# sunshinnnn/DSMnet

Measured on AMD Instinct MI355X. Metric: stereo pairs/sec forward, PSMNet D=192 384×1280, at 1/2/4/8 MI355X, higher is better.
Workload: dtype f32

## Files before the change

### dsmnet_amd/_lib.py

```python
import ctypes
import os

_HERE = os.path.dirname(os.path.abspath(__file__))
LIB_PATH = os.environ.get("DSM_LIB_PATH") or os.path.join(_HERE, "csrc", "libdsmnet_hip.so")

c_int, c_void_p, c_size_t = ctypes.c_int, ctypes.c_void_p, ctypes.c_size_t

DSM_OK = 0
DSM_F32 = 0
DSM_NCDHW, DSM_NDHWC = 0, 1
DSM_CONV_FP32_MFMA, DSM_CONV_COUT1_CHUNKED, DSM_CONV_TM_SHIFT, DSM_CONV_BLOCKS_SHIFT = 1, 2, 4, 16
DSM_CONV_NO_NSPLIT = 4
DSM_CONV_NO_ONCE = 8
DSM_PREC_F32, DSM_PREC_F16, DSM_PREC_F16X2 = 0, 1, 2


class Bn3dArgs(ctypes.Structure):
    _fields_ = [("y", c_void_p), ("residual", c_void_p), ("out", c_void_p), ("gamma", c_void_p),
                ("beta", c_void_p), ("running_mean", c_void_p), ("running_var", c_void_p),
                ("affine", c_void_p), ("workspace", c_void_p), ("gout", c_void_p), ("dy", c_void_p),
                ("dresidual", c_void_p), ("B", c_int), ("C", c_int),
                ("Dy", c_int), ("Hy", c_int), ("Wy", c_int), ("Dr", c_int), ("Hr", c_int), ("Wr", c_int),
                ("relu", c_int), ("momentum", ctypes.c_float), ("eps", ctypes.c_float),
                ("out_amax", c_void_p), ("dy_amax", c_void_p), ("dres_amax", c_void_p)]


class Conv3dArgs(ctypes.Structure):
    _fields_ = [("x", c_void_p), ("w_packed", c_void_p), ("scale", c_void_p),
                ("shift", c_void_p), ("residual", c_void_p), ("y", c_void_p),
                ("B", c_int), ("Cin", c_int), ("Cout", c_int),
                ("Di", c_int), ("Hi", c_int), ("Wi", c_int),
                ("Do", c_int), ("Ho", c_int), ("Wo", c_int),
                ("Dr", c_int), ("Hr", c_int), ("Wr", c_int),
                ("stride", c_int), ("transposed", c_int), ("relu", c_int),
                ("kd", c_int), ("k", c_int), ("dil", c_int),
                ("flags", c_int), ("precision", c_int), ("x_amax", c_void_p), ("y_amax", c_void_p),
                ("vol_virtual", c_int), ("vol_mask_left", c_int)]


class BasicBlock2dArgs(ctypes.Structure):
    _fields_ = [("x", c_void_p), ("y", c_void_p), ("w1_packed", c_void_p), ("w2_packed", c_void_p),
                ("scale1", c_void_p), ("shift1", c_void_p), ("scale2", c_void_p), ("shift2", c_void_p),
                ("x_amax", c_void_p), ("y_amax", c_void_p),
                ("B", c_int), ("H", c_int), ("W", c_int), ("C", c_int), ("precision", c_int), ("relu", c_int), ("no_skip", c_int)]


# ... 72 lines not shown
```

### dsmnet_amd/csrc/build.py

```python
import os
import subprocess
import sys
from concurrent.futures import ThreadPoolExecutor

HERE = os.path.dirname(os.path.abspath(__file__))
SOURCES = ["abi.hip", "corr1d.hip", "cost_volume.hip", "soft_argmin.hip", "conv3d.hip", "conv_f16.hip",
           "conv3d_bwd.hip", "bn3d.hip", "decoder.hip", "spp.hip", "warp.hip"]
LIB = os.path.join(HERE, "libdsmnet_hip.so")
HIPCC = os.environ.get("HIPCC", "/opt/rocm/bin/hipcc")
FLAGS = ["--offload-arch=gfx950", "-O3", "-std=c++17", "-fPIC",
         "-Wall", "-Wno-unused-function"] + os.environ.get("HIPCC_EXTRA", "").split()


def _stale(out, deps):
    if not os.path.exists(out):
        return True
    t = os.path.getmtime(out)
    return any(os.path.getmtime(d) > t for d in deps)


def build(force=False, verbose=True, stamps=False):
    if stamps:
        lib = os.path.join(HERE, "libdsmnet_hip_stamps.so")
        srcs = [os.path.join(HERE, s) for s in SOURCES]
        extra = ["-DDSM_ABLATE=%s" % os.environ["DSM_ABLATE"]] if os.environ.get("DSM_ABLATE") else []
        cmd = [HIPCC] + FLAGS + ["-DDSM_STAMPS"] + extra + ["-shared", "-o", lib] + srcs
        print(" ".join(cmd), flush=True)
        subprocess.run(cmd, check=True)
        return lib
    hdrs = [os.path.join(HERE, "common.hpp"), os.path.join(HERE, "conv_split.hpp"), os.path.join(HERE, "conv_zs.hpp"), os.path.join(HERE, "conv_common.hpp"),
            os.path.join(HERE, "..", "..", "include", "dsmnet_hip.h")]
    srcs = [os.path.join(HERE, s) for s in SOURCES if os.path.exists(os.path.join(HERE, s))]
    objs = []
    jobs = []
    for s in srcs:
        o = s[:-4] + ".o"
        objs.append(o)
        if force or _stale(o, [s] + hdrs):
            jobs.append([HIPCC] + FLAGS + ["-c", s, "-o", o])

    def run(cmd):
        if verbose:
            print(" ".join(cmd), flush=True)
        r = subprocess.run(cmd, capture_output=True, text=True)
        if r.returncode != 0:
            raise RuntimeError("hipcc failed:\n%s\n%s" % (r.stdout, r.stderr))
        if verbose and r.stderr.strip():
            print(r.stderr)

    with ThreadPoolExecutor(max_workers=min(4, max(1, len(jobs)))) as ex:
        list(ex.map(run, jobs))
    if jobs or force or _stale(LIB, objs):
        run([HIPCC, "--offload-arch=gfx950", "-shared", "-fPIC", "-o", LIB] + objs)
    return LIB


if __name__ == "__main__":
    print(build(force="--force" in sys.argv, stamps="--stamps" in sys.argv))
```

### dsmnet_amd/csrc/conv3d.hip

```cpp
#include "conv_common.hpp"

#ifdef DSM_STAMPS
__device__ unsigned long long dsm_stamp_buf[8 * 1024];
#define DSM_STAMP(slot)                                                                  \
  do {                                                                                   \
    __builtin_amdgcn_sched_barrier(0);                                                   \
    unsigned long long _t;                                                               \
    asm volatile("s_memtime %0\n\ts_waitcnt lgkmcnt(0)" : "=s"(_t)::"memory");           \
    __builtin_amdgcn_sched_barrier(0);                                                   \
    if (threadIdx.x == 0 && blockIdx.x < 1024) dsm_stamp_buf[blockIdx.x * 8 + (slot)] += _t - _tprev; \
    _tprev = _t;                                                                         \
  } while (0)
#define DSM_STAMP_INIT()                                                                 \
  unsigned long long _tprev;                                                             \
  asm volatile("s_memtime %0\n\ts_waitcnt lgkmcnt(0)" : "=s"(_tprev)::"memory")
extern "C" int dsm_debug_read_stamps(unsigned long long* host, int zero) {
  if (hipMemcpyFromSymbol(host, HIP_SYMBOL(dsm_stamp_buf), sizeof(unsigned long long) * 8 * 1024) != hipSuccess) return -3;
  if (zero) {
    static unsigned long long z[8 * 1024];
    if (hipMemcpyToSymbol(HIP_SYMBOL(dsm_stamp_buf), z, sizeof(z)) != hipSuccess) return -3;
  }
  return 0;
}
#else
// ... 895 lines not shown
    return DSM_OK;
  }
  if (a->stride == 2 && kd == 3 && NT == 2 && bf16x3_enabled(a) &&
      4l * a->B * a->Di * a->Hi * a->Wi * a->Cin < 0x80000000l) {
    *pl = Plan{5, 2, 2, 1, 16, 3, 3, 1};
    return DSM_OK;
  }
fp32_kernels:
  if (kd == 1) {
    const int TM = (big && NT == 1 && a->stride == 1 && k == 3 && dil == 1) ? 2 : 1;
    *pl = Plan{0, a->stride, NT, TM, 16, 1, k, dil};
    return DSM_OK;
  }
  if (a->stride == 1) {
    const int force_tm = forced_tm(a) <= 2 ? forced_tm(a) : 0;
    const int TM = force_tm ? force_tm : ((big && NT <= 2) ? 2 : 1);
    *pl = Plan{0, 1, NT, TM, (NT == 2 && TM == 2) ? 8 : 16, 3, 3, 1};
  } else {
    *pl = Plan{0, 2, NT, 1, 8, 3, 3, 1};
  }
  const long tiles4 = (long)a->B * a->Do * dsm_cdiv(a->Ho, 4) * dsm_cdiv(a->Wo, 32);
  if (NT >= 2 && tiles4 <= 64 && pl->TM == 1) { pl->nsplit = NT; pl->NT = 1; }
  return DSM_OK;
}
int make_plan(const dsm_conv3d_args* a, Plan* pl) {
  const int rc = make_plan_f32(a, pl);
  if (rc != DSM_OK) return rc;
  pl->pm = 3;
  if ((pl->kind == 5 || pl->kind == 6 || pl->kind == 7) && a->precision != DSM_PREC_F32) {
    DSM_REQUIRE(a->x_amax != nullptr, DSM_ERR_ARG);
    pl->pm = a->precision == DSM_PREC_F16X2 ? 2 : 1;
  }
  if (pl->pm == 3) pl->once = 0;
  return DSM_OK;
}
}

extern "C" int dsm_conv3d_plan(const dsm_conv3d_args* a, char* buf, int len) {
  DSM_REQUIRE(buf && len > 0, DSM_ERR_ARG);
  Plan pl;
  int rc = make_plan(a, &pl);
  if (rc != DSM_OK) { buf[0] = 0; return rc; }
  switch (pl.kind) {
    case 0:
      if (pl.KZ == 3 && pl.nsplit > 1) snprintf(buf, len, "conv3d_mfma_kernel<S=%d,NT=%d,TM=%d,CK=%d>x%d", pl.S, pl.NT, pl.TM, pl.CK, pl.nsplit);
      else if (pl.KZ == 3) snprintf(buf, len, "conv3d_mfma_kernel<S=%d,NT=%d,TM=%d,CK=%d>", pl.S, pl.NT, pl.TM, pl.CK);
      else snprintf(buf, len, "conv2d_mfma_kernel<S=%d,NT=%d,TM=%d,K=%d,DIL=%d>", pl.S, pl.NT, pl.TM, pl.K, pl.DIL);
      break;
    case 1: snprintf(buf, len, "deconv3d_mfma_kernel<NT=%d,CK=%d>", pl.NT, pl.CK); break;
    case 2: snprintf(buf, len, "conv3d_cout1_kernel<CK=%d>", pl.CK); break;
    case 4: snprintf(buf, len, "conv3d_cout1_zslide_kernel"); break;
    case 5: {
      const char* pr = pl.pm == 3 ? "bf16x3" : (pl.pm == 2 ? "f16x2" : "f16");
      if (pl.KZ == 3 && pl.S == 2) snprintf(buf, len, "conv3d_%s_mfma_kernel<S=2,NT=%d,TM=%d>", pr, pl.NT, pl.TM);
      else if (pl.KZ == 3 && pl.nsplit > 1) snprintf(buf, len, "conv3d_%s_mfma_kernel<NT=%d,TM=%d>x%d", pr, pl.NT, pl.TM, pl.nsplit);
      else if (pl.KZ == 3) snprintf(buf, len, "conv3d_%s_mfma_kernel<NT=%d,TM=%d>", pr, pl.NT, pl.TM);
      else if (pl.once) snprintf(buf, len, "conv2d_%s_mfma_kernel<NT=%d,TM=%d,DIL=%d>x%d,once", pr, pl.NT, pl.TM, pl.DIL, pl.nsplit);
      else if (pl.nsplit > 1) snprintf(buf, len, "conv2d_%s_mfma_kernel<NT=%d,TM=%d,DIL=%d>x%d", pr, pl.NT, pl.TM, pl.DIL, pl.nsplit);
      else snprintf(buf, len, "conv2d_%s_mfma_kernel<NT=%d,TM=%d,DIL=%d>", pr, pl.NT, pl.TM, pl.DIL);
      break;
    }
    case 7: snprintf(buf, len, "conv3d_zs_%s_mfma_kernel%s", pl.pm == 3 ? "bf16x3" : (pl.pm == 2 ? "f16x2" : "f16"), a->vol_virtual ? "<vol>" : ""); break;
    case 6: snprintf(buf, len, "deconv3d_%s_mfma_kernel<NT=%d>", pl.pm == 3 ? "bf16x3" : (pl.pm == 2 ? "f16x2" : "f16"), pl.NT); break;
    default: snprintf(buf, len, "deconv3d_cout1_kernel"); break;
  }
  return DSM_OK;
}

extern "C" int dsm_basicblock2d_fwd(const dsm_basicblock2d_args* a, dsm_stream_t stream) {
  DSM_REQUIRE(a && a->x && a->y && a->w1_packed && a->w2_packed && a->x_amax, DSM_ERR_ARG);
  DSM_REQUIRE((a->C == 64 || a->C == 32) && a->B > 0 && a->H > 0 && a->W > 0, DSM_ERR_UNSUPPORTED);
  DSM_REQUIRE(a->precision == DSM_PREC_F16X2 || a->precision == DSM_PREC_F16, DSM_ERR_UNSUPPORTED);
  DSM_REQUIRE(a->relu == 0 || a->relu == 1, DSM_ERR_ARG);
  const int C = a->C;
  const unsigned long xb = 4ul * a->B * a->H * a->W * C;
  DSM_REQUIRE(xb < 0x80000000ul, DSM_ERR_UNSUPPORTED);
  const size_t sec3 = (size_t)C * C * 9 * 4 + bf16x3_section_bytes(C, C, 1, 3);
  BbParams p;
  p.x = (const float*)a->x; p.y = (float*)a->y;
  p.w1_amax = (const float*)((const char*)a->w1_packed + sec3);
  p.w2_amax = (const float*)((const char*)a->w2_packed + sec3);
  p.w1 = (const unsigned char*)a->w1_packed + sec3 + 16;
  p.w2 = (const unsigned char*)a->w2_packed + sec3 + 16;
  p.scale1 = a->scale1; p.shift1 = a->shift1; p.scale2 = a->scale2; p.shift2 = a->shift2;
  p.x_amax = a->x_amax; p.y_amax = a->y_amax;
  p.B = a->B; p.H = a->H; p.W = a->W; p.C = C; p.relu = a->relu; p.skip = a->no_skip ? 0 : 1; p.ntx = p.nty = p.ntiles = 0;
  p.xbytes = (unsigned)xb;
  p.wbytes = (unsigned)(f16_section_bytes(C, C, 1, 3) - 16);
  dsm_clear_stale_error();
  return dsmk::run_basicblock_f16(a->precision == DSM_PREC_F16X2 ? 2 : 1, p, (hipStream_t)stream);
}

extern "C" int dsm_conv3d_fwd(const dsm_conv3d_args* a, dsm_stream_t stream) {
  Plan pl;
  int rc = make_plan(a, &pl);
  if (rc != DSM_OK) return rc;
// ... 12 lines not shown
    const size_t n = (size_t)a->Cin * 32 * 27;
    const char* sec2 = (const char*)a->w_packed + n * 4;
    const char* sec3 = sec2 + n * 6;
    z.x = (const float*)a->x; z.scale = a->scale; z.shift = a->shift; z.res = (const float*)a->residual;
    z.y = (float*)a->y; z.x_amax = a->x_amax; z.y_amax = a->y_amax;
    z.w_amax = pl.pm == 3 ? nullptr : (const float*)sec3;
    z.w = (const unsigned char*)(pl.pm == 3 ? sec2 : sec3 + 16);
    z.wbytes = (unsigned)(pl.pm == 3 ? n * 6 : n * 4);
    z.B = a->B; z.Cin = a->Cin;
    z.Di = a->Di; z.Hi = a->Hi; z.Wi = a->Wi; z.Do = a->Do; z.Ho = a->Ho; z.Wo = a->Wo;
    z.Dr = a->Dr; z.Hr = a->Hr; z.Wr = a->Wr; z.relu = a->relu;
    z.vol = a->vol_virtual ? 1 : 0; z.vol_mask_left = a->vol_mask_left ? 1 : 0;
    dsm_clear_stale_error();
    if (pl.pm == 3) return launch_conv_zs<3>(z, p.force_blocks, (hipStream_t)stream);
    return dsmk::run_zs_f16(pl.pm, z, p.force_blocks, (hipStream_t)stream);
  }
  {
    const unsigned long xb = 4ul * a->B * a->Di * a->Hi * a->Wi * a->Cin;
    const int kd_ = a->kd ? a->kd : 3, k_ = a->k ? a->k : 3;
    const unsigned long wb = 4ul * a->Cin * a->Cout * kd_ * k_ * k_;
    DSM_REQUIRE(xb < (1ul << 32) && wb < (1ul << 32), DSM_ERR_UNSUPPORTED);
    p.xbytes = (unsigned)xb; p.wbytes = (unsigned)wb;
  }
  hipStream_t s = (hipStream_t)stream;
  dsm_clear_stale_error();
  if (pl.kind == 3) {
    p.ntx = dsm_cdiv(p.Wi, 32); p.nty = dsm_cdiv(p.Hi, 4);
    const long nt = (long)p.B * p.Di * p.nty * p.ntx;
    DSM_REQUIRE(nt < (1L << 31), DSM_ERR_UNSUPPORTED);
    const size_t lds = (size_t)(2 * 5 * 33 * 8 + 27 * 8) * 16;
    hipLaunchKernelGGL(deconv3d_cout1_kernel, dim3((unsigned)nt), dim3(NTHREADS), lds, s, p);
    return dsm_launch_status();
  }
  if (pl.kind == 5 || pl.kind == 6) {
    const int kz = pl.kind == 6 ? 3 : pl.KZ;
    const char* sec2 = (const char*)a->w_packed + (size_t)a->Cin * a->Cout * kz * 9 * 4;
    if (pl.pm == 3) {
      p.w = (const float*)sec2;
      p.wbytes = (unsigned)bf16x3_section_bytes(a->Cin, a->Cout, kz, 3);
      return dispatch_split<3>(pl, p, s);
    }
    const char* sec3 = sec2 + bf16x3_section_bytes(a->Cin, a->Cout, kz, 3);
    p.w_amax = (const float*)sec3;
    p.w = (const float*)(sec3 + 16);
    p.wbytes = (unsigned)(f16_section_bytes(a->Cin, a->Cout, kz, 3) - 16);
    return dsmk::run_split_f16(pl, p, s);
  }
  if (pl.kind == 4) {
    p.ntx = dsm_cdiv(p.Wo, 32); p.nty = dsm_cdiv(p.Ho, 8);
    const long cols = (long)p.B * p.nty * p.ntx;
    int zseg = 16;
    while (zseg > 2 && cols * dsm_cdiv(p.Do, zseg) < 600) zseg >>= 1;
    const long nt = cols * dsm_cdiv(p.Do, zseg);
    DSM_REQUIRE(nt < (1L << 31), DSM_ERR_UNSUPPORTED);
    const size_t lds = (size_t)10 * 34 * 9 * 16;
    hipLaunchKernelGGL(conv3d_cout1_zslide_kernel, dim3((unsigned)nt), dim3(NTHREADS), lds, s, p,
                       p.w, zseg);
    return dsm_launch_status();
  }
  if (pl.kind == 2) {
    p.ntx = dsm_cdiv(p.Wo, 32); p.nty = dsm_cdiv(p.Ho, 8);
    p.ntiles = p.B * p.Do * p.nty * p.ntx;
    const size_t lds = (size_t)3 * 10 * 34 * 2 * 16;
    const int blocks = p.ntiles < 1024 ? p.ntiles : 1024;
    hipLaunchKernelGGL(conv3d_cout1_kernel<8>, dim3(blocks), dim3(NTHREADS), lds, s, p, p.w);
    return dsm_launch_status();
  }
#define DSM_CASE2D(S_, NT_, TM_, K_, DIL_) \
  if (pl.kind == 0 && pl.KZ == 1 && pl.S == S_ && pl.NT == NT_ && pl.TM == TM_ && pl.K == K_ && \
      pl.DIL == DIL_) return run_conv<S_, NT_, TM_, 16, 1, K_, DIL_>(p, s)
  DSM_CASE2D(1, 1, 1, 3, 1); DSM_CASE2D(1, 1, 2, 3, 1); DSM_CASE2D(1, 2, 1, 3, 1);
  DSM_CASE2D(1, 4, 1, 3, 1); DSM_CASE2D(1, 4, 1, 3, 2);
  DSM_CASE2D(2, 1, 1, 3, 1); DSM_CASE2D(2, 2, 1, 3, 1);
  DSM_CASE2D(1, 1, 1, 1, 1); DSM_CASE2D(1, 4, 1, 1, 1); DSM_CASE2D(2, 2, 1, 1, 1);
#undef DSM_CASE2D
  if (pl.KZ == 1) return DSM_ERR_UNSUPPORTED;
#define DSM_CASE(KIND, S_, NT_, TM_, CK_, CALL) \
  if (pl.kind == KIND && pl.S == S_ && pl.NT == NT_ && pl.TM == TM_ && pl.CK == CK_) return CALL
// ... 14 lines not shown
```

### dsmnet_amd/csrc/conv_common.hpp

```cpp
#pragma once
#include "common.hpp"
#include <type_traits>

namespace dsmk {

struct ConvParams {
  const float* x; const float* w; const float* scale; const float* shift;
  const float* res; float* y;
  int force_blocks;
  int single_kind;
  int B, Cin, Cout;
  int Di, Hi, Wi, Do, Ho, Wo, Dr, Hr, Wr;
  int relu;
  int ntx, nty, ntiles;
  unsigned xbytes, wbytes;
  int ntp;
  const float* x_amax; const float* w_amax;
  float* y_amax;
};

struct Plan { int kind; int S, NT, TM, CK; int KZ, K, DIL; int nsplit = 1; int pm = 3; int once = 0; };

struct ZsParams {
  const float* x;
  const unsigned char* w;
  const float* scale; const float* shift;
  const float* res;
  float* y;
  const float* x_amax; const float* w_amax; float* y_amax;
  int B, Cin;
  int Di, Hi, Wi, Do, Ho, Wo, Dr, Hr, Wr;
  int relu;
  int vol, vol_mask_left;
  int ntx, nty, ncol;
  long nunits;
  unsigned wbytes;
};

__attribute__((visibility("hidden"))) int run_split_f16(const Plan& pl, const ConvParams& p, hipStream_t s);
__attribute__((visibility("hidden"))) int run_zs_f16(int pm, const ZsParams& p, int grid, hipStream_t s);

struct BbParams {
  const float* x; float* y;
  const unsigned char* w1; const unsigned char* w2;
  const float* w1_amax; const float* w2_amax;
  const float* scale1; const float* shift1; const float* scale2; const float* shift2;
  const float* x_amax; float* y_amax;
  int B, H, W, C, relu, skip, ntx, nty, ntiles;
  unsigned xbytes, wbytes;
};

__attribute__((visibility("hidden"))) int run_basicblock_f16(int pm, const BbParams& p, hipStream_t s);

}

namespace {

using dsmk::ConvParams;
using dsmk::Plan;
using dsmk::ZsParams;
using dsmk::BbParams;

template <int I, int N, typename F>
__device__ __forceinline__ void static_for(F&& f) {
  if constexpr (I < N) {
    f(std::integral_constant<int, I>{});
    static_for<I + 1, N>(f);
  }
}

constexpr int NTHREADS = 256;

template <int S, int KZ = 3, int KXY = 3, int DIL = 1> struct Geo {
// ... 143 lines not shown
```

### dsmnet_amd/csrc/conv_f16.hip

```cpp
#include "conv_common.hpp"

namespace {
#include "conv_split.hpp"
#include "conv_zs.hpp"
#include "basicblock2d.hpp"
}

int dsmk::run_zs_f16(int pm, const ZsParams& p, int grid, hipStream_t s) {
  if (pm == 2) return launch_conv_zs<2>(p, grid, s);
  if (pm == 1) return launch_conv_zs<1>(p, grid, s);
  return DSM_ERR_UNSUPPORTED;
}

int dsmk::run_split_f16(const Plan& pl, const ConvParams& p, hipStream_t s) {
  if (pl.pm == 2) return dispatch_split<2>(pl, p, s);
  if (pl.pm == 1) return dispatch_split<1>(pl, p, s);
  return DSM_ERR_UNSUPPORTED;
}

int dsmk::run_basicblock_f16(int pm, const BbParams& p, hipStream_t s) {
  if (pm == 2) return p.C == 64 ? launch_basicblock2d<2, 64>(p, s) : launch_basicblock2d<2, 32>(p, s);
  if (pm == 1) return p.C == 64 ? launch_basicblock2d<1, 64>(p, s) : launch_basicblock2d<1, 32>(p, s);
  return DSM_ERR_UNSUPPORTED;
}
```

### include/dsmnet_hip.h

```cpp
#ifndef DSMNET_HIP_H
#define DSMNET_HIP_H

#include <stddef.h>
#include <stdint.h>

#ifdef __cplusplus
extern "C" {
#endif

#define DSM_ABI_VERSION 7

#define DSM_OK               0
#define DSM_ERR_ARG         -1
#define DSM_ERR_UNSUPPORTED -2
#define DSM_ERR_LAUNCH      -3
#define DSM_ERR_ALIGN       -4

enum dsm_dtype  { DSM_F32 = 0 };
enum dsm_layout { DSM_NCDHW = 0, DSM_NDHWC = 1 };

typedef void* dsm_stream_t;

int         dsm_abi_version(void);
const char* dsm_strerror(int code);
// ... 25 lines not shown
                        int negate, int align_corners, int dtype, dsm_stream_t stream);

typedef struct dsm_conv3d_args {
  const void*  x;
  const void*  w_packed;
  const float* scale;
  const float* shift;
  const void*  residual;
  void*        y;
  int B, Cin, Cout;
  int Di, Hi, Wi;
  int Do, Ho, Wo;
  int Dr, Hr, Wr;
  int stride;
  int transposed;
  int relu;
  int kd;
  int k;
  int dil;
  int          flags;
  int          precision;
  const float* x_amax;
  float*       y_amax;
  int          vol_virtual;
  int          vol_mask_left;
} dsm_conv3d_args;
#define DSM_PREC_F32    0
#define DSM_PREC_F16    1
#define DSM_PREC_F16X2  2
#define DSM_CONV_FP32_MFMA      0x1
#define DSM_CONV_COUT1_CHUNKED  0x2
#define DSM_CONV_NO_NSPLIT      0x4
#define DSM_CONV_NO_ONCE        0x8
#define DSM_CONV_TM_SHIFT       4
#define DSM_CONV_BLOCKS_SHIFT   16

size_t dsm_conv3d_packed_weight_bytes(int Cin, int Cout, int transposed);

int dsm_conv3d_pack_weights(const void* w_torch, void* w_packed,
                            int Cin, int Cout, int transposed, dsm_stream_t stream);

size_t dsm_conv_packed_weight_bytes(int Cin, int Cout, int kd, int k);
int dsm_conv_pack_weights(const void* w_torch, void* w_packed, int Cin_src, int Cin, int Cout,
                          int kd, int k, dsm_stream_t stream);

int dsm_absmax(const void* x, size_t n, float* amax, dsm_stream_t stream);

typedef struct {
  const void* x; void* y;
  const void* w1_packed; const void* w2_packed;
  const float* scale1; const float* shift1; const float* scale2; const float* shift2;
  const float* x_amax; float* y_amax;
  int B, H, W, C;
  int precision;
  int relu;
  int no_skip;
} dsm_basicblock2d_args;
int dsm_basicblock2d_fwd(const dsm_basicblock2d_args* a, dsm_stream_t stream);

int dsm_conv3d_fwd(const dsm_conv3d_args* args, dsm_stream_t stream);

int dsm_conv3d_plan(const dsm_conv3d_args* args, char* buf, int len);

int dsm_conv3d_wgrad(const void* x, const void* g, void* ws, void* dw, int B, int Cx, int Cg,
                     int Dx, int Hx, int Wx, int Dg, int Hg, int Wg, int stride, int flags,
                     int precision, const float* x_amax, const float* g_amax, dsm_stream_t stream);
// ... 64 lines not shown
```

Measured before the change: 201.5.

## Add warp-specialized persistent 2D conv kernel for Cout=128 f16 MFMA path

```diff
diff --git a/dsmnet_amd/_lib.py b/dsmnet_amd/_lib.py
--- a/dsmnet_amd/_lib.py
+++ b/dsmnet_amd/_lib.py
@@ -12,6 +12,7 @@
 DSM_CONV_FP32_MFMA, DSM_CONV_COUT1_CHUNKED, DSM_CONV_TM_SHIFT, DSM_CONV_BLOCKS_SHIFT = 1, 2, 4, 16
 DSM_CONV_NO_NSPLIT = 4
 DSM_CONV_NO_ONCE = 8
+DSM_CONV_NO_T128 = 0x100
 DSM_PREC_F32, DSM_PREC_F16, DSM_PREC_F16X2 = 0, 1, 2
 
 
diff --git a/dsmnet_amd/csrc/build.py b/dsmnet_amd/csrc/build.py
--- a/dsmnet_amd/csrc/build.py
+++ b/dsmnet_amd/csrc/build.py
@@ -1,3 +1,4 @@
+import glob
 import os
 import subprocess
 import sys
@@ -28,8 +29,7 @@
         print(" ".join(cmd), flush=True)
         subprocess.run(cmd, check=True)
         return lib
-    hdrs = [os.path.join(HERE, "common.hpp"), os.path.join(HERE, "conv_split.hpp"), os.path.join(HERE, "conv_zs.hpp"), os.path.join(HERE, "conv_common.hpp"),
-            os.path.join(HERE, "..", "..", "include", "dsmnet_hip.h")]
+    hdrs = sorted(glob.glob(os.path.join(HERE, "*.hpp"))) + [os.path.join(HERE, "..", "..", "include", "dsmnet_hip.h")]
     srcs = [os.path.join(HERE, s) for s in SOURCES if os.path.exists(os.path.join(HERE, s))]
     objs = []
     jobs = []
diff --git a/dsmnet_amd/csrc/conv3d.hip b/dsmnet_amd/csrc/conv3d.hip
--- a/dsmnet_amd/csrc/conv3d.hip
+++ b/dsmnet_amd/csrc/conv3d.hip
@@ -951,6 +951,10 @@
     pl->pm = a->precision == DSM_PREC_F16X2 ? 2 : 1;
   }
   if (pl->pm == 3) pl->once = 0;
+  if (pl->pm != 3 && pl->kind == 5 && pl->KZ == 1 && pl->S == 1 && a->Cout == 128 && a->Cin % 32 == 0 &&
+      a->Cin >= 96 && !(a->flags & DSM_CONV_NO_T128)) {
+    pl->kind = 8; pl->NT = 4; pl->TM = 2; pl->nsplit = 1; pl->once = 0;
+  }
   return DSM_OK;
 }
 }
@@ -979,6 +983,7 @@
       else snprintf(buf, len, "conv2d_%s_mfma_kernel<NT=%d,TM=%d,DIL=%d>", pr, pl.NT, pl.TM, pl.DIL);
       break;
     }
+    case 8: snprintf(buf, len, "conv2d_%s_mfma_t128_kernel<DIL=%d>", pl.pm == 2 ? "f16x2" : "f16", pl.DIL); break;
     case 7: snprintf(buf, len, "conv3d_zs_%s_mfma_kernel%s", pl.pm == 3 ? "bf16x3" : (pl.pm == 2 ? "f16x2" : "f16"), a->vol_virtual ? "<vol>" : ""); break;
     case 6: snprintf(buf, len, "deconv3d_%s_mfma_kernel<NT=%d>", pl.pm == 3 ? "bf16x3" : (pl.pm == 2 ? "f16x2" : "f16"), pl.NT); break;
     default: snprintf(buf, len, "deconv3d_cout1_kernel"); break;
@@ -1059,7 +1064,7 @@
     hipLaunchKernelGGL(deconv3d_cout1_kernel, dim3((unsigned)nt), dim3(NTHREADS), lds, s, p);
     return dsm_launch_status();
   }
-  if (pl.kind == 5 || pl.kind == 6) {
+  if (pl.kind == 5 || pl.kind == 6 || pl.kind == 8) {
     const int kz = pl.kind == 6 ? 3 : pl.KZ;
     const char* sec2 = (const char*)a->w_packed + (size_t)a->Cin * a->Cout * kz * 9 * 4;
     if (pl.pm == 3) {
@@ -1071,6 +1076,7 @@
     p.w_amax = (const float*)sec3;
     p.w = (const float*)(sec3 + 16);
     p.wbytes = (unsigned)(f16_section_bytes(a->Cin, a->Cout, kz, 3) - 16);
+    if (pl.kind == 8) return dsmk::run_t128_f16(pl.pm, pl.DIL, p, s);
     return dsmk::run_split_f16(pl, p, s);
   }
   if (pl.kind == 4) {
diff --git a/dsmnet_amd/csrc/conv_common.hpp b/dsmnet_amd/csrc/conv_common.hpp
--- a/dsmnet_amd/csrc/conv_common.hpp
+++ b/dsmnet_amd/csrc/conv_common.hpp
@@ -39,6 +39,7 @@
 
 __attribute__((visibility("hidden"))) int run_split_f16(const Plan& pl, const ConvParams& p, hipStream_t s);
 __attribute__((visibility("hidden"))) int run_zs_f16(int pm, const ZsParams& p, int grid, hipStream_t s);
+__attribute__((visibility("hidden"))) int run_t128_f16(int pm, int dil, const ConvParams& p, hipStream_t s);
 
 struct BbParams {
   const float* x; float* y;
diff --git a/dsmnet_amd/csrc/conv_f16.hip b/dsmnet_amd/csrc/conv_f16.hip
--- a/dsmnet_amd/csrc/conv_f16.hip
+++ b/dsmnet_amd/csrc/conv_f16.hip
@@ -3,6 +3,7 @@
 namespace {
 #include "conv_split.hpp"
 #include "conv_zs.hpp"
+#include "conv_t128.hpp"
 #include "basicblock2d.hpp"
 }
 
@@ -18,6 +19,12 @@
   return DSM_ERR_UNSUPPORTED;
 }
 
+int dsmk::run_t128_f16(int pm, int dil, const ConvParams& p, hipStream_t s) {
+  if (pm == 2) return dil == 1 ? run_conv_t128<2, 1>(p, s) : run_conv_t128<2, 2>(p, s);
+  if (pm == 1) return dil == 1 ? run_conv_t128<1, 1>(p, s) : run_conv_t128<1, 2>(p, s);
+  return DSM_ERR_UNSUPPORTED;
+}
+
 int dsmk::run_basicblock_f16(int pm, const BbParams& p, hipStream_t s) {
   if (pm == 2) return p.C == 64 ? launch_basicblock2d<2, 64>(p, s) : launch_basicblock2d<2, 32>(p, s);
   if (pm == 1) return p.C == 64 ? launch_basicblock2d<1, 64>(p, s) : launch_basicblock2d<1, 32>(p, s);
diff --git a/dsmnet_amd/csrc/conv_t128.hpp b/dsmnet_amd/csrc/conv_t128.hpp
--- /dev/null
+++ b/dsmnet_amd/csrc/conv_t128.hpp
@@ -0,0 +1,251 @@
+#pragma once
+
+#ifndef DSM_T128_OFF
+#define DSM_T128_OFF 0
+#endif
+
+template <int PM, int DIL> struct T128Cfg {
+  static constexpr int NP = Prec<PM>::NP, NPW = Prec<PM>::NPW;
+  static constexpr int THREADS = 512, NSTAGE = 256;
+  static constexpr int TY = 8, CK = 16, NTP = 4, COUT = 128;
+  static constexpr int IY = TY + 2 * DIL, IX = 32 + 2 * DIL;
+  static constexpr int NVOX = IY * IX;
+  static constexpr int NE = NVOX * 4;
+  static constexpr int NPF = (NE + NSTAGE - 1) / NSTAGE;
+  static constexpr int PITCH = 32 * NP + 16;
+  static constexpr int IMG = NPF * 64 * PITCH;
+  static constexpr int LDS = 2 * IMG + 2 * COUT * 4;
+  static constexpr int NITEM = 9;
+  static constexpr int WRING = PM == 1 ? 9 : 3, WAHEAD = PM == 1 ? 5 : 2;
+  static constexpr int XR = 4;
+  static_assert(NITEM % WRING == 0 && WAHEAD < WRING, "weight ring");
+  static_assert(LDS <= 160 * 1024, "LDS");
+};
+
+template <int PM, int DIL>
+__global__ __launch_bounds__(512, 1) void conv_t128_kernel(ConvParams p) {
+  using C = T128Cfg<PM, DIL>;
+  using frag = typename Prec<PM>::frag;
+  constexpr int NP = C::NP, NPW = C::NPW, TY = C::TY, CK = C::CK, IX = C::IX, NE = C::NE, NPF = C::NPF,
+                PITCH = C::PITCH, IMG = C::IMG, NTP = C::NTP, COUT = C::COUT, NITEM = C::NITEM,
+                WRING = C::WRING, WAHEAD = C::WAHEAD, XR = C::XR;
+  constexpr int NGROUP = NITEM * TY;
+  extern __shared__ __attribute__((aligned(16))) unsigned char lds_raw[];
+  const int tid = threadIdx.x, lane = tid & 63, wave = tid >> 6;
+  const bool staging = wave >= 4;
+  const int nch = p.Cin / CK;
+
+  const int G = gridDim.x, id = blockIdx.x;
+  const int logical = (G & 7) == 0 ? (id & 7) * (G >> 3) + (id >> 3) : id;
+  const int t_begin = (int)((long)p.ntiles * logical / G), t_end = (int)((long)p.ntiles * (logical + 1) / G);
+  if (t_begin >= t_end) return;
+
+  const SplitScale ss = split_scale<PM>(p);
+  float* const aff = reinterpret_cast<float*>(lds_raw + 2 * IMG);
+  for (int i = tid; i < 2 * COUT; i += C::THREADS)
+    aff[i] = i < COUT ? (p.scale ? p.scale[i] * ss.out : ss.out) : (p.shift ? p.shift[i - COUT] : 0.f);
+  float am = 0.f;
+
+  struct Pos { int t, ck; bool valid; };
+  auto advance = [&](Pos q) {
+    if (++q.ck == nch) { q.ck = 0; ++q.t; }
+    q.valid = q.t < t_end;
+    return q;
+  };
+  const Pos first = {t_begin, 0, true};
+
+  if (staging) {
+    const int st = tid - C::NSTAGE;
+    constexpr unsigned OOBV = 0x80000000u;
+    unsigned goff[NPF], yx[NPF], voff[NPF];
+#pragma unroll
+    for (int k = 0; k < NPF; ++k) {
+      const int e = st + k * C::NSTAGE;
+      const int v = e / 4, q = e % 4;
+      const int yy = v / IX, xx = v % IX;
+      goff[k] = 4u * (unsigned)((yy * p.Wi + xx) * p.Cin + 4 * q);
+      yx[k] = e < NE ? ((unsigned)yy << 16 | (unsigned)xx) : 0x7fff0000u;
+    }
+    auto tile_offsets = [&](int t) {
+      const int tx = t % p.ntx, ty = (t / p.ntx) % p.nty, b = t / (p.ntx * p.nty);
+      const int yb = ty * TY - DIL, xb = tx * 32 - DIL;
+      const unsigned base = (unsigned)(4l * ((((long)b * p.Hi + yb) * p.Wi + xb) * p.Cin));
+#pragma unroll
+      for (int k = 0; k < NPF; ++k) {
+        const int y = yb + (int)(yx[k] >> 16), x = xb + (int)(yx[k] & 0xffffu);
+        const bool ok = (unsigned)y < (unsigned)p.Hi && (unsigned)x < (unsigned)p.Wi;
+        voff[k] = ok ? base + goff[k] : OOBV;
+      }
+    };
+    f32x4 pf[2][NPF];
+    auto load_chunk = [&](auto setc, const Pos& c) {
+      constexpr int set = decltype(setc)::value;
+      const unsigned sh = (unsigned)c.ck * (CK * 4);
+      const __amdgpu_buffer_rsrc_t rs =
+          make_rsrc(reinterpret_cast<const char*>(p.x) + sh, c.valid ? p.xbytes - sh : 0u);
+#pragma unroll
+      for (int k = 0; k < NPF; ++k) pf[set][k] = buffer_load16(rs, voff[k], 0);
+    };
+    const int wr_off = (st >> 2) * PITCH + (st & 3) * 8;
+    auto split_chunk = [&](auto setc, unsigned char* img) {
+      constexpr int set = decltype(setc)::value;
+#pragma unroll
+      for (int k = 0; k < NPF; ++k) {
+        unsigned lo[NP], hi[NP];
+        split_pair<PM>(pf[set][k].x, pf[set][k].y, ss.sx, lo);
+        split_pair<PM>(pf[set][k].z, pf[set][k].w, ss.sx, hi);
+#pragma unroll
+        for (int q = 0; q < NP; ++q) {
+          u32x2 v; v.x = lo[q]; v.y = hi[q];
+          *reinterpret_cast<u32x2*>(img + wr_off + k * (64 * PITCH) + q * 32) = v;
+        }
+      }
+    };
+
+    constexpr std::integral_constant<int, 0> S0{};
+    constexpr std::integral_constant<int, 1> S1{};
+    Pos c0 = first;
+    tile_offsets(c0.t);
+    load_chunk(S0, c0);
+    split_chunk(S0, lds_raw);
+    Pos c1 = advance(c0);
+    if (c1.valid && c1.t != c0.t) tile_offsets(c1.t);
+    load_chunk(S1, c1);
+    __syncthreads();
+    auto iteration = [&](auto parc) {
+      constexpr int P = decltype(parc)::value;
+      const Pos c2 = advance(c1);
+#if DSM_T128_OFF & 2
+      if (p.B == 12345) {
+#endif
+      if (c2.valid && c2.t != c1.t) tile_offsets(c2.t);
+      load_chunk(parc, c2);
+      if (c1.valid) split_chunk(std::integral_constant<int, P ^ 1>{}, lds_raw + (P ^ 1) * IMG);
+#if DSM_T128_OFF & 2
+      }
+#endif
+      __syncthreads();
+      c0 = c1; c1 = c2;
+      return !c0.valid;
+    };
+    while (true) {
+      if (iteration(S0)) break;
+      if (iteration(S1)) break;
+    }
+  } else {
+    const int n = wave, r = lane & 31, h = lane >> 5;
+    const __amdgpu_buffer_rsrc_t wrsrc = make_rsrc(p.w, p.wbytes);
+    const unsigned lane16 = lane * 16u + (unsigned)n * (NPW * 1024);
+    constexpr unsigned WTAP = NTP * NPW * 1024;
+    const int rd_off = r * PITCH + h * 16;
+    f32x16 acc[TY];
+    frag wq[WRING][NP];
+    frag xq[XR][NP];
+    auto zero_acc = [&]() {
+#pragma unroll
+      for (int m = 0; m < TY; ++m)
+#pragma unroll
+        for (int i = 0; i < 16; ++i) acc[m][i] = 0.f;
+    };
+    auto wload = [&](auto ic, unsigned wb) {
+      constexpr int item = decltype(ic)::value;
+#pragma unroll
+      for (int q = 0; q < NP; ++q)
+        wq[item % WRING][q] = __builtin_bit_cast(frag, buffer_load16(wrsrc, lane16, wb + item * WTAP + q * 1024));
+    };
+    auto xload = [&](auto sc, const unsigned char* rd) {
+      constexpr int s = decltype(sc)::value;
+      constexpr int item = s / TY, m = s % TY;
+      constexpr int vo = (m + (item / 3) * DIL) * IX + (item % 3) * DIL;
+#pragma unroll
+      for (int q = 0; q < NP; ++q) xq[s % XR][q] = *reinterpret_cast<const frag*>(rd + vo * PITCH + q * 32);
+    };
+    auto epilogue = [&](int t) {
+      const int tx0 = (t % p.ntx) * 32, ty0 = ((t / p.ntx) % p.nty) * TY, tb = t / (p.ntx * p.nty);
+      const int xo = tx0 + r;
+      if (xo >= p.Wo) return;
+      const int cbase = n * 32 + 4 * h;
+      const Affine af = load_affine_lds(aff, COUT, cbase);
+      constexpr int RB = 2;
+#pragma unroll
+      for (int m0 = 0; m0 < TY; m0 += RB) {
+        Residual rr[RB];
+        if (p.res) {
+#pragma unroll
+          for (int mi = 0; mi < RB; ++mi) {
+            const int yo = ty0 + m0 + mi;
+            if (yo >= p.Ho) continue;
+            load_residual(rr[mi], p.res + (((long)tb * p.Dr * p.Hr + yo) * p.Wr + xo) * COUT + cbase);
+          }
+        }
+#pragma unroll
+        for (int mi = 0; mi < RB; ++mi) {
+          const int yo = ty0 + m0 + mi;
+          if (yo >= p.Ho) continue;
+#if DSM_T128_OFF & 1
+          if (p.B != 12345) continue;
+#endif
+          store_tile<COUT>(acc[m0 + mi], af, p.relu, p.y + (((long)tb * p.Do * p.Ho + yo) * p.Wo + xo) * COUT + cbase,
+                           rr[mi], p.res != nullptr, am);
+        }
+      }
+    };
+
+    Pos cur = first;
+    zero_acc();
+    static_for<0, WAHEAD>([&](auto ic) { wload(ic, 0u); });
+    int i = 0;
+    __syncthreads();
+    while (true) {
+      const unsigned char* const rd = lds_raw + (i & 1) * IMG + rd_off;
+      const Pos nxt = advance(cur);
+      const unsigned wcur = (unsigned)cur.ck * (NITEM * WTAP);
+      const unsigned wnext = nxt.valid ? (unsigned)nxt.ck * (NITEM * WTAP) : wcur;
+      static_for<0, XR - 1>([&](auto sc) { xload(sc, rd); });
+      __builtin_amdgcn_sched_barrier(0);
+      static_for<0, NITEM>([&](auto ic) {
+        constexpr int item = decltype(ic)::value;
+        if constexpr (item + WAHEAD < NITEM) wload(std::integral_constant<int, item + WAHEAD>{}, wcur);
+        else wload(std::integral_constant<int, item + WAHEAD - NITEM>{}, wnext);
+        static_for<0, TY>([&](auto mc) {
+          constexpr int m = decltype(mc)::value;
+          constexpr int s = item * TY + m;
+          if constexpr (s + XR - 1 < NGROUP) xload(std::integral_constant<int, s + XR - 1>{}, rd);
+          __builtin_amdgcn_sched_barrier(0);
+          mma32<PM>(acc[m], wq[item % WRING], xq[s % XR]);
+          __builtin_amdgcn_sched_barrier(0);
+        });
+      });
+      if (cur.ck == nch - 1) {
+        epilogue(cur.t);
+        zero_acc();
+      }
+      __syncthreads();
+      cur = nxt; ++i;
+      if (!cur.valid) break;
+    }
+  }
+  flush_amax8(p.y_amax, am, reinterpret_cast<float*>(lds_raw));
+}
+
+template <int PM, int DIL>
+int run_conv_t128(ConvParams p, hipStream_t s) {
+  using C = T128Cfg<PM, DIL>;
+  if (p.Cin % 32 != 0 || p.Cin < 64 || p.Cout != C::COUT || p.Di != 1 || p.Do != 1) return DSM_ERR_UNSUPPORTED;
+  if (p.xbytes >= 0x80000000u) return DSM_ERR_UNSUPPORTED;
+  p.ntx = dsm_cdiv(p.Wo, 32); p.nty = dsm_cdiv(p.Ho, C::TY);
+  const long nt = (long)p.B * p.nty * p.ntx;
+  if (nt >= (1L << 30)) return DSM_ERR_UNSUPPORTED;
+  p.ntiles = (int)nt;
+  static thread_local bool configured = false;
+  if (!configured) {
+    if (hipFuncSetAttribute((const void*)conv_t128_kernel<PM, DIL>, hipFuncAttributeMaxDynamicSharedMemorySize,
+                            C::LDS) != hipSuccess)
+      return DSM_ERR_LAUNCH;
+    configured = true;
+  }
+  int blocks = p.force_blocks ? p.force_blocks : 256;
+  if (blocks > p.ntiles) blocks = p.ntiles;
+  hipLaunchKernelGGL((conv_t128_kernel<PM, DIL>), dim3(blocks), dim3(C::THREADS), C::LDS, s, p);
+  return dsm_launch_status();
+}
diff --git a/include/dsmnet_hip.h b/include/dsmnet_hip.h
--- a/include/dsmnet_hip.h
+++ b/include/dsmnet_hip.h
@@ -81,6 +81,7 @@
 #define DSM_CONV_COUT1_CHUNKED  0x2
 #define DSM_CONV_NO_NSPLIT      0x4
 #define DSM_CONV_NO_ONCE        0x8
+#define DSM_CONV_NO_T128        0x100
 #define DSM_CONV_TM_SHIFT       4
 #define DSM_CONV_BLOCKS_SHIFT   16
 
```

New measurement: 201.3 (median of 2 runs). Within noise of the previous version (-0.1%).

## Add warp-specialized z-sliding deconv3d kernel for reduced-precision transposed convs

Applied to the files above, without the earlier changes.

```diff
diff --git a/dsmnet_amd/csrc/build.py b/dsmnet_amd/csrc/build.py
--- a/dsmnet_amd/csrc/build.py
+++ b/dsmnet_amd/csrc/build.py
@@ -28,7 +28,7 @@
         print(" ".join(cmd), flush=True)
         subprocess.run(cmd, check=True)
         return lib
-    hdrs = [os.path.join(HERE, "common.hpp"), os.path.join(HERE, "conv_split.hpp"), os.path.join(HERE, "conv_zs.hpp"), os.path.join(HERE, "conv_common.hpp"),
+    hdrs = [os.path.join(HERE, "common.hpp"), os.path.join(HERE, "conv_split.hpp"), os.path.join(HERE, "conv_zs.hpp"), os.path.join(HERE, "deconv_zs.hpp"), os.path.join(HERE, "conv_common.hpp"),
             os.path.join(HERE, "..", "..", "include", "dsmnet_hip.h")]
     srcs = [os.path.join(HERE, s) for s in SOURCES if os.path.exists(os.path.join(HERE, s))]
     objs = []
diff --git a/dsmnet_amd/csrc/conv3d.hip b/dsmnet_amd/csrc/conv3d.hip
--- a/dsmnet_amd/csrc/conv3d.hip
+++ b/dsmnet_amd/csrc/conv3d.hip
@@ -951,6 +951,9 @@
     pl->pm = a->precision == DSM_PREC_F16X2 ? 2 : 1;
   }
   if (pl->pm == 3) pl->once = 0;
+  if (pl->kind == 6 && pl->pm != 3 && DSM_DECONV_ZS && a->Cin % 64 == 0 &&
+      4l * a->Hi * a->Wi * a->Cin < 0x7fffffffl)
+    pl->zs = 1;
   return DSM_OK;
 }
 }
@@ -980,7 +983,8 @@
       break;
     }
     case 7: snprintf(buf, len, "conv3d_zs_%s_mfma_kernel%s", pl.pm == 3 ? "bf16x3" : (pl.pm == 2 ? "f16x2" : "f16"), a->vol_virtual ? "<vol>" : ""); break;
-    case 6: snprintf(buf, len, "deconv3d_%s_mfma_kernel<NT=%d>", pl.pm == 3 ? "bf16x3" : (pl.pm == 2 ? "f16x2" : "f16"), pl.NT); break;
+    case 6: snprintf(buf, len, "deconv3d_%s%s_mfma_kernel<NT=%d>", pl.zs ? "zs_" : "",
+                     pl.pm == 3 ? "bf16x3" : (pl.pm == 2 ? "f16x2" : "f16"), pl.NT); break;
     default: snprintf(buf, len, "deconv3d_cout1_kernel"); break;
   }
   return DSM_OK;
diff --git a/dsmnet_amd/csrc/conv_common.hpp b/dsmnet_amd/csrc/conv_common.hpp
--- a/dsmnet_amd/csrc/conv_common.hpp
+++ b/dsmnet_amd/csrc/conv_common.hpp
@@ -19,7 +19,11 @@
   float* y_amax;
 };
 
-struct Plan { int kind; int S, NT, TM, CK; int KZ, K, DIL; int nsplit = 1; int pm = 3; int once = 0; };
+struct Plan { int kind; int S, NT, TM, CK; int KZ, K, DIL; int nsplit = 1; int pm = 3; int once = 0; int zs = 0; };
+
+#ifndef DSM_DECONV_ZS
+#define DSM_DECONV_ZS 1
+#endif
 
 struct ZsParams {
   const float* x;
diff --git a/dsmnet_amd/csrc/conv_f16.hip b/dsmnet_amd/csrc/conv_f16.hip
--- a/dsmnet_amd/csrc/conv_f16.hip
+++ b/dsmnet_amd/csrc/conv_f16.hip
@@ -3,6 +3,7 @@
 namespace {
 #include "conv_split.hpp"
 #include "conv_zs.hpp"
+#include "deconv_zs.hpp"
 #include "basicblock2d.hpp"
 }
 
@@ -13,6 +14,7 @@
 }
 
 int dsmk::run_split_f16(const Plan& pl, const ConvParams& p, hipStream_t s) {
+  if (pl.kind == 6 && pl.zs) return pl.pm == 2 ? run_deconv_zs<2>(p, s) : run_deconv_zs<1>(p, s);
   if (pl.pm == 2) return dispatch_split<2>(pl, p, s);
   if (pl.pm == 1) return dispatch_split<1>(pl, p, s);
   return DSM_ERR_UNSUPPORTED;
diff --git a/dsmnet_amd/csrc/deconv_zs.hpp b/dsmnet_amd/csrc/deconv_zs.hpp
--- /dev/null
+++ b/dsmnet_amd/csrc/deconv_zs.hpp
@@ -0,0 +1,378 @@
+#pragma once
+
+
+template <int PM> struct DzsCfg {
+  static constexpr int NP = Prec<PM>::NP, NPW = Prec<PM>::NPW;
+  static constexpr int THREADS = 512, NSTAGE = 256;
+  static constexpr int TY = 2, IY = TY + 1, IX = 33;
+  static constexpr int NV = IY * IX;
+  static constexpr int NPF = (NV * 8 + NSTAGE - 1) / NSTAGE;
+  static constexpr int NVP = 32 * NPF;
+  static constexpr int ROW = NVP * 16;
+  static constexpr int IMG = NP * 4 * ROW;
+  static constexpr int XPL = 2 * TY * 64 * 8 * 16;
+  static constexpr int LDS = 2 * IMG + 2 * XPL;
+  static constexpr int NSTEP = 27;
+#ifndef DSM_DZS_DEPTH
+#define DSM_DZS_DEPTH 4
+#endif
+  static constexpr int DEPTH = DSM_DZS_DEPTH;
+  static_assert(DEPTH == 2 || DEPTH == 4, "the staging loop is unrolled four times");
+  static constexpr int WRING = 9, WAHEAD = 8;
+  static_assert(NSTEP % WRING == 0 && WAHEAD < WRING, "weight ring");
+  static_assert(LDS <= 160 * 1024, "LDS");
+};
+
+template <int PM>
+__global__ __launch_bounds__(512, 1) void deconv_zs_kernel(ConvParams p) {
+  using C = DzsCfg<PM>;
+  using T = ZsTerms<PM>;
+  using frag = typename Prec<PM>::frag;
+  constexpr int NP = C::NP, NPW = C::NPW, TY = C::TY, IX = C::IX, NV = C::NV, NPF = C::NPF, ROW = C::ROW,
+                IMG = C::IMG, XPL = C::XPL, NSTEP = C::NSTEP, WRING = C::WRING, WAHEAD = C::WAHEAD;
+  extern __shared__ __attribute__((aligned(16))) unsigned char lds_raw[];
+  const int tid = threadIdx.x, lane = tid & 63, wave = tid >> 6;
+  const bool staging = wave >= 4;
+  const int w4 = wave & 3;
+  const int ncg = p.Cin >> 5;
+  const int NTP = p.Cout >> 5;
+  const int MD = (p.Do + 1) >> 1;
+
+  const int G = gridDim.x, id = blockIdx.x;
+  const int logical = (G & 7) == 0 ? (id & 7) * (G >> 3) + (id >> 3) : id;
+  const long nunits = (long)p.ntiles * MD;
+  const long u_begin = nunits * logical / G, u_end = nunits * (logical + 1) / G;
+  if (u_begin >= u_end) return;
+
+  float sx = 1.f, so = 1.f;
+  {
+    const int ex = dsm_amax_exponent(*p.x_amax), ew = dsm_amax_exponent(*p.w_amax);
+    sx = __builtin_bit_cast(float, __builtin_amdgcn_readfirstlane(__builtin_bit_cast(int, dsm_pow2f(ex))));
+    so = dsm_pow2f(-(ex + ew));
+  }
+  unsigned char* const xch = lds_raw + 2 * IMG;
+  float am = 0.f;
+
+  struct It { long u; int col, m0, m1, zhi, zi, cg; bool valid; };
+  auto open_segment = [&](long u) {
+    It q; q.u = u; q.valid = u < u_end;
+    if (!q.valid) { q.col = q.m0 = q.m1 = q.zhi = q.zi = q.cg = 0; return q; }
+    q.col = (int)(u / MD); q.m0 = (int)(u % MD);
+    q.m1 = (int)min((long)MD, (long)q.m0 + (u_end - u));
+    q.zhi = 2 * q.m1 - 1 < p.Do ? q.m1 : q.m1 - 1;
+    q.zi = q.m0; q.cg = 0;
+    return q;
+  };
+  auto advance = [&](It q) {
+    if (++q.cg < ncg) return q;
+    q.cg = 0;
+    if (++q.zi <= q.zhi) return q;
+    return open_segment(q.u + (q.m1 - q.m0));
+  };
+  auto handover = [&](const It& q) {
+    if (!q.valid || q.cg != ncg - 1) return 0u;
+    unsigned m = 0;
+    if (q.zi - 1 >= q.m0 && q.zi - 1 < q.m1 && 2 * q.zi - 1 < p.Do) m |= 1u;
+    if (q.zi >= q.m0 && q.zi < q.m1) m |= 2u;
+    return m;
+  };
+
+  if (staging) {
+    const int stid = tid & 255;
+    const unsigned vstride = (unsigned)p.Cin * 4u;
+    const unsigned plane_bytes = vstride * (unsigned)p.Hi * (unsigned)p.Wi;
+    constexpr unsigned OOBV = 0x80000000u;
+    const int sq = 2 * (lane >> 4) + (lane & 1), sv = 8 * w4 + ((lane & 15) >> 1);
+    unsigned voff[NPF];
+    auto column_offsets = [&](int col) {
+      const int t = col / NTP;
+      const int y0 = ((t / p.ntx) % p.nty) * TY, x0 = (t % p.ntx) * 32;
+#pragma unroll
+      for (int k = 0; k < NPF; ++k) {
+        const int v = sv + 32 * k;
+        const int y = y0 + v / IX, x = x0 + v % IX;
+        const bool ok = v < NV && y < p.Hi && x < p.Wi;
+        voff[k] = ok ? ((unsigned)y * (unsigned)p.Wi + (unsigned)x) * vstride + 16u * (unsigned)sq : OOBV;
+      }
+    };
+    f32x4 pf[C::DEPTH][NPF];
+    auto load_chunk = [&](auto setc, const It& q) {
+      constexpr int set = decltype(setc)::value;
+      const int b = (q.col / NTP) / (p.ntx * p.nty);
+      const bool live = q.valid && q.zi < p.Di;
+      const long off = live ? ((long)b * p.Di + q.zi) * (long)plane_bytes + (long)q.cg * 128 : 0;
+      const __amdgpu_buffer_rsrc_t rs = make_rsrc(reinterpret_cast<const char*>(p.x) + off, live ? plane_bytes : 0u);
+#pragma unroll
+      for (int k = 0; k < NPF; ++k) pf[set][k] = buffer_load16(rs, voff[k], 0);
+    };
+    const int st_off = (lane >> 4) * ROW + sv * 16 + (lane & 1) * 8;
+    auto split_chunk = [&](auto setc, unsigned char* wr) {
+      constexpr int set = decltype(setc)::value;
+#pragma unroll
+      for (int k = 0; k < NPF; ++k) {
+        unsigned lo[NP], hi[NP];
+        split_pair<PM>(pf[set][k].x, pf[set][k].y, sx, lo);
+        split_pair<PM>(pf[set][k].z, pf[set][k].w, sx, hi);
+#pragma unroll
+        for (int q = 0; q < NP; ++q) {
+          u32x2 v; v.x = lo[q]; v.y = hi[q];
+          *reinterpret_cast<u32x2*>(wr + q * 4 * ROW + 512 * k) = v;
+        }
+      }
+    };
+    const int qd = stid & 7, ev = stid >> 3;
+    f32x4 sc[2], sh[2];
+#pragma unroll
+    for (int nb = 0; nb < 2; ++nb) {
+      const int c = 32 * (nb < NTP ? nb : 0) + 4 * qd;
+#pragma unroll
+      for (int e = 0; e < 4; ++e) {
+        sc[nb][e] = p.scale ? p.scale[c + e] * so : so;
+        sh[nb][e] = p.shift ? p.shift[c + e] : 0.f;
+      }
+    }
+    struct Pend { int col, zi; unsigned m; };
+    struct Where { int b, Y0, X0, nb; };
+    auto where = [&](int col) {
+      Where q;
+      const int t = col / NTP;
+      q.nb = col - t * NTP;
+      q.b = t / (p.ntx * p.nty);
+      q.Y0 = 2 * (((t / p.ntx) % p.nty) * TY);
+      q.X0 = 2 * ((t % p.ntx) * 32);
+      return q;
+    };
+    f32x4 resq[2][8];
+#pragma unroll
+    for (int s = 0; s < 2; ++s)
+#pragma unroll
+      for (int k = 0; k < 8; ++k) resq[s][k] = f32x4{0.f, 0.f, 0.f, 0.f};
+    auto vmask_of = [&](const Where& q) {
+      unsigned m = 0;
+#pragma unroll
+      for (int k = 0; k < 8; ++k)
+        if (q.Y0 + (k >> 1) < p.Ho && q.X0 + ev + 32 * (k & 1) < p.Wo) m |= 1u << k;
+      return m;
+    };
+    auto load_res = [&](const Pend& e) __attribute__((always_inline)) {
+      if (!e.m || !p.res) return;
+      const Where q = where(e.col);
+      const unsigned vm = vmask_of(q);
+#pragma unroll
+      for (int s = 0; s < 2; ++s) {
+        if (!((e.m >> s) & 1u)) continue;
+        const float* const rb = p.res + ((((long)q.b * p.Dr + 2 * e.zi - 1 + s) * p.Hr + q.Y0) * p.Wr + q.X0 + ev) * p.Cout +
+                                32 * q.nb + 4 * qd;
+#pragma unroll
+        for (int k = 0; k < 8; ++k)
+          if ((vm >> k) & 1u)
+            resq[s][k] = *reinterpret_cast<const f32x4*>(rb + ((k >> 1) * p.Wr + 32 * (k & 1)) * p.Cout);
+      }
+    };
+    const float lo2 = p.relu == 2 ? 0.f : -__builtin_huge_valf(), lo1 = p.relu == 1 ? 0.f : -__builtin_huge_valf();
+    auto vmax = [](f32x4 v, float lo) {
+      v.x = fmaxf(v.x, lo); v.y = fmaxf(v.y, lo); v.z = fmaxf(v.z, lo); v.w = fmaxf(v.w, lo);
+      return v;
+    };
+    auto epilogue = [&](const Pend& e) __attribute__((always_inline)) {
+      if (!e.m) return;
+      const Where q = where(e.col);
+      const unsigned vm = vmask_of(q);
+      const f32x4 s_ = q.nb ? sc[1] : sc[0], h_ = q.nb ? sh[1] : sh[0];
+#pragma unroll
+      for (int s = 0; s < 2; ++s) {
+        if (!((e.m >> s) & 1u)) continue;
+        f32x4 v[8];
+#pragma unroll
+        for (int k = 0; k < 8; ++k) {
+          const int oy = k >> 1, ox = ev + 32 * (k & 1);
+          v[k] = *reinterpret_cast<const f32x4*>(xch + s * XPL + ((oy * 64 + ox) * 8 + (qd ^ ((ox >> 1) & 7))) * 16);
+        }
+        float* const yb = p.y + ((((long)q.b * p.Do + 2 * e.zi - 1 + s) * p.Ho + q.Y0) * p.Wo + q.X0 + ev) * p.Cout +
+                          32 * q.nb + 4 * qd;
+#pragma unroll
+        for (int k = 0; k < 8; ++k) {
+          if (!((vm >> k) & 1u)) continue;
+          f32x4 o = vmax(v[k] * s_ + h_, lo2);
+          if (p.res) o += resq[s][k];
+          o = vmax(o, lo1);
+          *reinterpret_cast<f32x4*>(yb + ((k >> 1) * p.Wo + 32 * (k & 1)) * p.Cout) = o;
+          track_amax(am, o);
+        }
+      }
+    };
+
+    constexpr int D = C::DEPTH;
+    It c0 = open_segment(u_begin);
+    It lead = c0;
+    column_offsets(c0.col);
+    load_chunk(std::integral_constant<int, 0>{}, lead);
+    split_chunk(std::integral_constant<int, 0>{}, lds_raw + st_off);
+    static_for<1, D>([&](auto dc) {
+      const It nl = advance(lead);
+      if (nl.valid && nl.col != lead.col) column_offsets(nl.col);
+      lead = nl;
+      load_chunk(dc, lead);
+    });
+    It c1 = advance(c0);
+    Pend pend = {0, 0, 0u};
+    load_res(Pend{c0.col, c0.zi, handover(c0)});
+    __syncthreads();
+    auto iteration = [&](auto pc) {
+      constexpr int P = decltype(pc)::value;
+      const It nl = advance(lead);
+      if (nl.valid && nl.col != lead.col) column_offsets(nl.col);
+      lead = nl;
+      load_chunk(std::integral_constant<int, P % D>{}, lead);
+      if (c1.valid) split_chunk(std::integral_constant<int, (P + 1) % D>{}, lds_raw + ((P + 1) & 1) * IMG + st_off);
+      epilogue(pend);
+      pend = Pend{c0.col, c0.zi, handover(c0)};
+      load_res(Pend{c1.col, c1.zi, handover(c1)});
+      __syncthreads();
+      c0 = c1; c1 = advance(c1);
+      return !c0.valid;
+    };
+    while (true) {
+      if (iteration(std::integral_constant<int, 0>{})) break;
+      if (iteration(std::integral_constant<int, 1>{})) break;
+      if (iteration(std::integral_constant<int, 2>{})) break;
+      if (iteration(std::integral_constant<int, 3>{})) break;
+    }
+    epilogue(pend);
+  } else {
+    const int j = lane & 15, kg = lane >> 4;
+    const int ah = w4 >> 1, xh = w4 & 1;
+    const unsigned tstride = (unsigned)NTP * (NPW * 1024);
+    const __amdgpu_buffer_rsrc_t wrsrc = make_rsrc(p.w, p.wbytes);
+    const unsigned wlane = (unsigned)(kg >> 1) * 27u * tstride + (unsigned)(32 * (kg & 1) + 16 * ah + j) * 16u;
+    auto wbase_of = [&](const It& q) {
+      return (unsigned)q.cg * 54u * tstride + (unsigned)(q.col % NTP) * (NPW * 1024);
+    };
+    const int rd_off = kg * ROW + (16 * xh + j) * 16;
+    f32x4 acc[3][4][TY];
+    frag xq[2][TY][NP];
+    frag wq[WRING][NP];
+    auto zero_set = [&](auto sc_) {
+      constexpr int s = decltype(sc_)::value;
+#pragma unroll
+      for (int c = 0; c < 4; ++c)
+#pragma unroll
+        for (int r = 0; r < TY; ++r) acc[s][c][r] = f32x4{0.f, 0.f, 0.f, 0.f};
+    };
+    auto wload = [&](auto sc_, unsigned wb) {
+      constexpr int s = decltype(sc_)::value;
+      constexpr int tap = (s % 3) * 9 + dc_tap9(s / 3);
+#pragma unroll
+      for (int q = 0; q < NP; ++q)
+        wq[s % WRING][q] = __builtin_bit_cast(frag, buffer_load16(wrsrc, wlane, wb + (unsigned)tap * tstride + q * 1024));
+    };
+    auto xload = [&](auto oc, const unsigned char* rd) {
+      constexpr int o = decltype(oc)::value, iy = o >> 1, ix = o & 1;
+#pragma unroll
+      for (int r = 0; r < TY; ++r)
+#pragma unroll
+        for (int q = 0; q < NP; ++q)
+          xq[o & 1][r][q] = *reinterpret_cast<const frag*>(rd + q * 4 * ROW + ((r + iy) * IX + ix) * 16);
+    };
+    auto zmask_of = [&](const It& q) {
+      unsigned m = 0;
+      if (q.zi >= q.m0 && q.zi < q.m1) m |= 6u;
+      if (q.zi - 1 >= q.m0 && q.zi - 1 < q.m1 && q.zi < p.Di && 2 * q.zi - 1 < p.Do) m |= 1u;
+      return m;
+    };
+    It cur = open_segment(u_begin);
+    static_for<0, 3>([&](auto s) { zero_set(s); });
+    static_for<0, WAHEAD>([&](auto sc_) { wload(sc_, wbase_of(cur)); });
+    int i = 0;
+    __syncthreads();
+    while (true) {
+      const unsigned char* const rd = lds_raw + (i & 1) * IMG + rd_off;
+      const It nxt = advance(cur);
+      const unsigned wcur = wbase_of(cur);
+      const unsigned wnext = nxt.valid ? wbase_of(nxt) : 0u;
+      const unsigned mask = zmask_of(cur);
+      xload(std::integral_constant<int, 0>{}, rd);
+      __builtin_amdgcn_sched_barrier(0);
+      static_for<0, NSTEP>([&](auto sc_) {
+        constexpr int s = decltype(sc_)::value;
+        constexpr int jp = s / 3, kz = s % 3;
+        constexpr DcPair pr = dc_pair(jp);
+        constexpr bool fresh = kz == 0 && (jp == 0 || jp == 4 || jp == 6 || jp == 8);
+        if constexpr (s + WAHEAD < NSTEP) wload(std::integral_constant<int, s + WAHEAD>{}, wcur);
+        else wload(std::integral_constant<int, s + WAHEAD - NSTEP>{}, wnext);
+        if constexpr (fresh && pr.o + 1 < 4) xload(std::integral_constant<int, pr.o + 1>{}, rd);
+        __builtin_amdgcn_sched_barrier(0);
+        if ((mask >> kz) & 1u) {
+          static_for<0, T::N>([&](auto tc) {
+            constexpr int t = decltype(tc)::value;
+            static_for<0, TY>([&](auto rc) {
+              constexpr int r = decltype(rc)::value;
+              acc[kz][pr.c][r] = zs_mfma<PM>(wq[s % WRING][T::w[t]], xq[pr.o & 1][r][T::x[t]], acc[kz][pr.c][r]);
+            });
+          });
+        }
+        __builtin_amdgcn_sched_barrier(0);
+      });
+      if (cur.cg == ncg - 1) {
+        const unsigned m = handover(cur);
+#pragma unroll
+        for (int s = 0; s < 2; ++s) {
+          if (!((m >> s) & 1u)) continue;
+#pragma unroll
+          for (int c = 0; c < 4; ++c)
+#pragma unroll
+            for (int r = 0; r < TY; ++r) {
+              const int oy = 2 * r + (c >> 1), ox = 2 * (16 * xh + j) + (c & 1);
+              const int unit = (oy * 64 + ox) * 8 + ((4 * ah + kg) ^ (j & 7));
+              *reinterpret_cast<f32x4*>(xch + s * XPL + unit * 16) = acc[s][c][r];
+            }
+        }
+#pragma unroll
+        for (int c = 0; c < 4; ++c)
+#pragma unroll
+          for (int r = 0; r < TY; ++r) acc[0][c][r] = acc[2][c][r];
+        zero_set(std::integral_constant<int, 1>{});
+        zero_set(std::integral_constant<int, 2>{});
+      }
+      __syncthreads();
+      cur = nxt; ++i;
+      if (!cur.valid) break;
+    }
+  }
+  if (p.y_amax) {
+#pragma unroll
+    for (int o = 32; o; o >>= 1) am = fmaxf(am, __shfl_xor(am, o));
+    float* const red = reinterpret_cast<float*>(lds_raw);
+    __syncthreads();
+    if (lane == 0) red[wave] = am;
+    __syncthreads();
+    if (tid == 0) {
+      am = fmaxf(fmaxf(fmaxf(red[0], red[1]), fmaxf(red[2], red[3])), fmaxf(fmaxf(red[4], red[5]), fmaxf(red[6], red[7])));
+      if (am > __builtin_nontemporal_load(p.y_amax))
+        atomicMax(reinterpret_cast<unsigned*>(p.y_amax), __builtin_bit_cast(unsigned, am));
+    }
+  }
+}
+
+template <int PM>
+int run_deconv_zs(ConvParams p, hipStream_t s) {
+  using C = DzsCfg<PM>;
+  DSM_REQUIRE(p.Cin % 64 == 0 && (p.Cout == 32 || p.Cout == 64) && 4l * p.Hi * p.Wi * p.Cin < 0x7fffffffl,
+              DSM_ERR_UNSUPPORTED);
+  p.ntx = dsm_cdiv(p.Wi, 32); p.nty = dsm_cdiv(p.Hi, C::TY);
+  const long ncol = (long)p.B * p.nty * p.ntx * (p.Cout / 32);
+  DSM_REQUIRE(ncol * p.Di < (1L << 30), DSM_ERR_UNSUPPORTED);
+  p.ntiles = (int)ncol;
+  const long nunits = ncol * ((p.Do + 1) / 2);
+  static thread_local bool configured = false;
+  if (!configured) {
+    if (hipFuncSetAttribute((const void*)deconv_zs_kernel<PM>, hipFuncAttributeMaxDynamicSharedMemorySize,
+                            C::LDS) != hipSuccess)
+      return DSM_ERR_LAUNCH;
+    configured = true;
+  }
+  int blocks = p.force_blocks ? p.force_blocks : 256;
+  if ((long)blocks > nunits) blocks = (int)nunits;
+  hipLaunchKernelGGL(deconv_zs_kernel<PM>, dim3(blocks), dim3(C::THREADS), C::LDS, s, p);
+  return dsm_launch_status();
+}
```

Result: faster. 195.6 before, 198.6 after (median of 6 runs) (+1.5%).
